# blepping/ComfyUI-sonar

Measured on AMD Instinct MI355X. Metric: noise-latents/sec (SDXL 4x128x128), higher is better.
Workload: dtype f32

## Files before the change

### comfyui-sonar_amd/csrc/power_fft.hip

```cpp
#include "power_core.h"

namespace sonar {

template <int H, int W>
constexpr int plane_min_waves() {
    return (H * W >= 32768 || (H == 256 && W == 64) || (H == 64 && W == 256) || (H == 64 && W == 32)) ? 2 : SONAR_FFT_WAVES;
}

template <int H, int W, int SRC, bool STATS, bool NORM>
__global__ void __launch_bounds__((plane_threads<H, W>()), (plane_min_waves<H, W>())) power_irfft2_kernel(const float* __restrict__ z,
                                                                       const float* __restrict__ filter, float* out,
                                                                       int64_t planes, uint64_t seed, uint64_t stream_id,
                                                                       int64_t plane_offset, int group, int split, double* partials,
                                                                       NormArgs na, StatsAhead sa) {
    kernarg_touch_for(z, filter, out, planes, seed, stream_id, plane_offset, group, split, partials, na, sa);
    using C = PlaneCfg<H, W>;
    constexpr int NT = plane_threads<H, W>();
    constexpr int M = C::M, S = C::S;
    constexpr int RN1 = C::RN1, RN2 = C::RN2;
    constexpr bool FAST = (W == 128) && (H == 128 || H == 64) && (NT == 512) && !SONAR_FFT_TW_LDS;
    constexpr int CN1 = FAST ? H / 8 : C::CN1, CN2 = FAST ? 8 : C::CN2;
    __shared__ c32 A[C::kLdsComplex];
    c32* const T0 = A + H * S;
    c32* const TM = T0 + H;
    c32* const TW = TM + H;
    __shared__ double red[2 * NT / 64];
    __shared__ NormDecision shd;
    __shared__ int edge_seq;
    constexpr bool kSumsInLds = SRC == 2 && STATS && FAST && H == 128;
    __shared__ double sums_lds[kSumsInLds ? 2 * NT : 1];
    const int tid = threadIdx.x;
    if constexpr (kSumsInLds) {
        sums_lds[tid] = 0.0;
        sums_lds[NT + tid] = 0.0;
    }
    int64_t bid = blockIdx.x, nblk = gridDim.x;
    if constexpr (SRC == 1 && NORM && !STATS) {
        static_assert(kStatsBatch * 2 * H <= C::kLdsComplex, "the statistics' edge columns borrow the plane's LDS");
        if (sa.partials) {
            if ((int)blockIdx.x >= sa.main_blocks) {
                power_stats_body<H, W>(filter, planes, seed, sa.stream_id, plane_offset, group, split, sa.partials, bid - sa.main_blocks,
                                       nblk - sa.main_blocks, reinterpret_cast<c32(*)[2][H]>(A), red);
                return;
            }
            nblk = sa.main_blocks;
        }
    }
    constexpr bool GEN = SRC == 1;
    float scale = SRC == 2 ? 1.0f / ((float)H * (float)W) : 1.0f / sqrtf((float)H * (float)W);
    float nm = scale, nc = 0.0f;
    constexpr int NPRE = (NORM && kNPart % NT == 0) ? kNPart / NT : 0;
    [[maybe_unused]] double pre_s[NPRE > 0 ? NPRE : 1], pre_q[NPRE > 0 ? NPRE : 1];
    [[maybe_unused]] bool norm_pending = NORM;
    if constexpr (NORM) {
        if constexpr (NPRE > 0) {
#pragma unroll
            for (int i = 0; i < NPRE; ++i) {
                pre_s[i] = na.partials[2 * (tid + i * NT)];
                pre_q[i] = na.partials[2 * (tid + i * NT) + 1];
            }
        } else {
            const NormDecision dec = decide_norm<NT>(na.partials, kNPart, na.n_total, na.thr_sd, red, &shd);
            const float g = (dec.do_div ? 1.0f / dec.stdv : 1.0f) * na.factor;
            nm = scale * g;
            nc = dec.do_sub ? dec.mean * g : 0.0f;
            norm_pending = false;
        }
    }
    double s = 0.0, q = 0.0;
    for (int j = tid; j < 256; j += NT) TW[j] = c_tw256[j];
#if SONAR_FFT_TW_LDS
    auto tw = [&](int idx, int n, bool) -> c32 { return TW[(idx * (256 / n)) & 255]; };
#else
    auto tw = [&] __device__(int idx, int n, bool uni) -> c32 {
        if (uni) return c_tw256[(__builtin_amdgcn_readfirstlane(idx) * (256 / n)) & 255];
        return TW[(idx * (256 / n)) & 255];
    };
#endif
    const int wv = __builtin_amdgcn_readfirstlane(tid >> 6);
    const int lane = tid & 63;
    c32 ctw[CN1], gtw[RN1], ptw[RN1];
    auto load_twiddles = [&] __device__(int w) {
#pragma unroll
        for (int k1 = 0; k1 < CN1; ++k1) ctw[k1] = c_tw256[((w * k1) * (256 / H)) & 255];
#pragma unroll
        for (int n1 = 0; n1 < RN1; ++n1) gtw[n1] = c_tw256[((RN2 * n1 + w) * (256 / W)) & 255];
#pragma unroll
        for (int k1 = 0; k1 < RN1; ++k1) ptw[k1] = c_tw256[((w * k1) * (256 / M)) & 255];
    };
    if constexpr (FAST) load_twiddles(wv);

#ifdef SONAR_PW_DESYNC
    if (blockIdx.x >= gridDim.x / 2)
        for (int i = 0; i < SONAR_PW_DESYNC; ++i) __builtin_amdgcn_s_sleep(32);
#endif
    [[maybe_unused]] int pidx = 0;
    [[maybe_unused]] int edge_want = 0;
    if (tid == 0) edge_seq = 0;
    for (int64_t unit = bid; unit < (split ? planes : planes / group); unit += nblk) {
    const GroupWalk gw(unit, group, split);
    SpectrumRng rng;
    if constexpr (GEN) {
        rng = spectrum_rng<H, true>(seed, stream_id, plane_offset / group + gw.grp, tid);
        for (int i = 0; i < gw.first; ++i) skip_plane<H, W, true>(rng, tid);
    }
    for (int gp = gw.first; gp < gw.first + gw.count; ++gp) {
        const int64_t plane = gw.grp * group + gp;
        __syncthreads();
        SONAR_STAMP(0);
        int ptid = tid;
        if constexpr (!FAST && H * W >= 4096) asm volatile("" : "+v"(ptid));
        if constexpr (SRC < 2) {
        auto sink = [&](int ky, int kx, c32 v) { (kx == 0 ? T0[ky] : kx == M ? TM[ky] : A[ky * S + kx]) = v; };
        __builtin_amdgcn_s_setprio(0);
        if constexpr (GEN) {
            if constexpr (!(SONAR_PW_SKIP & 1)) fill_plane_gen<H, W, S>(filter, rng, tid, A, T0, TM, (FAST && H == 2 * 64) ? &edge_seq : nullptr);
            if constexpr (FAST && H == 2 * 64 && !(SONAR_PW_SKIP & 1)) {
                edge_want += 2;
                if (tid >= NT - H) {
                    while (__hip_atomic_load(&edge_seq, __ATOMIC_RELAXED, __HIP_MEMORY_SCOPE_WORKGROUP) < edge_want) __builtin_amdgcn_s_sleep(1);
                    __builtin_amdgcn_fence(__ATOMIC_ACQUIRE, "workgroup");
                    const int ky = tid - (NT - H), kn = (H - ky) & (H - 1);
                    const c32 a = T0[ky], an = T0[kn], b = TM[ky], bn = TM[kn];
                    A[ky * S] = make_float2(0.5f * (a.x + an.x) - 0.5f * (b.y - bn.y), 0.5f * (a.y - an.y) + 0.5f * (b.x + bn.x));
                }
            }
        } else fill_plane<H, W>(z, filter, plane, tid, sink);
        __builtin_amdgcn_s_setprio(3);
        SONAR_STAMP(1);
        __syncthreads();
        SONAR_STAMP(2);
        } else {
        constexpr int Wh = M + 1;
        const float* const xin = z + plane * (int64_t)H * W;
#pragma unroll 2
        for (int item = ptid; item < RN1 * H; item += NT) {
            const int k1 = item % RN1, r = item / RN1;
            const int y = (r / CN2) + CN1 * (r % CN2);
            const float* xrow = xin + (int64_t)y * W;
            c32 u[RN2];
#pragma unroll
            for (int k2 = 0; k2 < RN2; ++k2) u[k2] = *reinterpret_cast<const float2*>(xrow + 2 * (k1 + RN1 * k2));
            fdft<RN2>(u);
#pragma unroll
            for (int n2 = 1; n2 < RN2; ++n2) u[n2] = cmulc(u[n2], tw(n2 * k1, M, false));
#pragma unroll
            for (int n2 = 0; n2 < RN2; ++n2) A[r * S + C::rpos(k1, n2)] = u[n2];
        }
        __syncthreads();
        {
            constexpr int ITEMS = (RN2 * H + NT - 1) / NT;
            c32 v[ITEMS][RN1];
#pragma unroll
// ... 191 lines not shown
#pragma unroll
                for (int n1 = 0; n1 < CN1; ++n1) v[n1] = A[(CN2 * n1 + n2) * S + c];
            } else {
#pragma unroll
                for (int n1 = 0; n1 < CN1; ++n1) {
                    const int ky = CN2 * n1 + n2, kn = (H - ky) & (H - 1);
                    const c32 a = T0[ky], an = T0[kn], b = TM[ky], bn = TM[kn];
                    v[n1] = make_float2(0.5f * (a.x + an.x) - 0.5f * (b.y - bn.y), 0.5f * (a.y - an.y) + 0.5f * (b.x + bn.x));
                }
            }
            idft<CN1>(v);
#pragma unroll
            for (int k1 = 1; k1 < CN1; ++k1) v[k1] = cmul(v[k1], tw(n2 * k1, H, M % 64 == 0));
#pragma unroll
            for (int k1 = 0; k1 < CN1; ++k1) A[(CN2 * k1 + n2) * S + c] = v[k1];
        }
        __syncthreads();
SONAR_UNROLL_ITEMS
        for (int item = ptid; item < CN1 * M; item += NT) {
            const int c = item % M, k1 = item / M;
            c32 u[CN2];
#pragma unroll
            for (int n2 = 0; n2 < CN2; ++n2) u[n2] = A[(CN2 * k1 + n2) * S + c];
            idft<CN2>(u);
#pragma unroll
            for (int k2 = 0; k2 < CN2; ++k2) A[(CN2 * k1 + k2) * S + c] = u[k2];
        }
        __syncthreads();
        {
            constexpr int ITEMS = (RN2 * H + NT - 1) / NT;
            c32 g[ITEMS][RN1];
#pragma unroll
            for (int it = 0; it < ITEMS; ++it) {
                const int item = ptid + it * NT;
                if (item < RN2 * H) {
                    const int r = item % H;
                    const int n2 = item / H;
                    const c32* row = A + r * S;
#pragma unroll
                    for (int n1 = 0; n1 < RN1; ++n1) {
                        const int k = RN2 * n1 + n2;
                        c32 xa, xb;
                        if (k == 0) {
                            const c32 p = row[0];
                            xa = make_float2(p.x, 0.0f);
                            xb = make_float2(p.y, 0.0f);
                        } else {
                            xa = row[k];
                            xb = row[M - k];
                        }
                        const c32 e = make_float2(xa.x + xb.x, xa.y - xb.y);
                        const c32 d = make_float2(xa.x - xb.x, xa.y + xb.y);
                        const c32 o = cmul(d, tw(k, W, H % 64 == 0));
                        g[it][n1] = make_float2(e.x - o.y, e.y + o.x);
                    }
                    idft<RN1>(g[it]);
#pragma unroll
                    for (int k1 = 1; k1 < RN1; ++k1) g[it][k1] = cmul(g[it][k1], tw(n2 * k1, M, H % 64 == 0));
                }
                __builtin_amdgcn_sched_barrier(0);
            }
            __syncthreads();
#pragma unroll
            for (int it = 0; it < ITEMS; ++it) {
                const int item = ptid + it * NT;
                if (item < RN2 * H) {
                    const int r = item % H;
                    const int n2 = item / H;
#pragma unroll
                    for (int k1 = 0; k1 < RN1; ++k1) A[r * S + C::rpos(k1, n2)] = g[it][k1];
                }
            }
        }
        __syncthreads();
        }
        if constexpr (NPRE > 0) {
            if (norm_pending) {
                double ps0 = 0.0, pq0 = 0.0;
#pragma unroll
                for (int i = 0; i < NPRE; ++i) {
                    ps0 += pre_s[i];
                    pq0 += pre_q[i];
                }
                const NormDecision dec = decide_from_sums<NT>(ps0, pq0, na.n_total, na.thr_sd, red, &shd);
                const float g = (dec.do_div ? 1.0f / dec.stdv : 1.0f) * na.factor;
                nm = scale * g;
                nc = dec.do_sub ? dec.mean * g : 0.0f;
                norm_pending = false;
            }
        }
        float* const oplane = out + plane * (int64_t)H * W;
        if constexpr (FAST && H == 128) {
            if constexpr (kSumsInLds) {
                double ps_ = 0.0, pq_ = 0.0;
                pipe_row_b<H, W, 8, STATS, NORM>(A, oplane, wv, lane, scale, nm, nc, ps_, pq_);
                sums_lds[tid] += ps_;
                sums_lds[NT + tid] += pq_;
            } else {
                pipe_row_b<H, W, 8, STATS, NORM>(A, oplane, wv, lane, scale, nm, nc, s, q);
            }
            SONAR_STAMP(11);
            ++pidx;
            continue;
        }
        float ps = 0.0f, pq = 0.0f;
SONAR_UNROLL_ITEMS
        for (int item = ptid; item < RN1 * H; item += NT) {
            const int k1 = item % RN1, r = item / RN1;
            const int y = (r / CN2) + CN1 * (r % CN2);
            c32 u[RN2];
#pragma unroll
            for (int n2 = 0; n2 < RN2; ++n2) u[n2] = (SONAR_PW_SKIP & 8) ? make_float2((float)(item + n2), 1.0f) : A[r * S + C::rpos(k1, n2)];
            if constexpr (!(SONAR_PW_SKIP & 8)) idft<RN2>(u);
            float* orow = oplane + (int64_t)y * W;
#pragma unroll
            for (int k2 = 0; k2 < RN2; ++k2) {
                float a, b;
                if constexpr (NORM) {
                    a = __builtin_fmaf(u[k2].x, nm, -nc);
                    b = __builtin_fmaf(u[k2].y, nm, -nc);
                } else {
                    a = u[k2].x * scale;
                    b = u[k2].y * scale;
                }
                if constexpr (!(SONAR_PW_SKIP & 16)) *reinterpret_cast<float2*>(orow + 2 * (k1 + RN1 * k2)) = make_float2(a, b);
                else if (a == 123.456f && b == 654.321f) *reinterpret_cast<float2*>(orow) = make_float2(a, b);
                if constexpr (STATS) {
                    ps += a + b;
                    pq = __builtin_fmaf(a, a, __builtin_fmaf(b, b, pq));
                }
            }
        }
        if constexpr (STATS) {
            s += (double)ps;
            q += (double)pq;
        }
        SONAR_STAMP(11);
        ++pidx;
    }
    }
    if constexpr (kSumsInLds) {
        s = sums_lds[tid];
        q = sums_lds[NT + tid];
    }
    if constexpr (STATS) write_partial<NT>(s, q, partials, red);
}

#ifndef SONAR_PIPE_NT
#define SONAR_PIPE_NT 0
#endif
#ifndef SONAR_PIPE_CHUNKS
#define SONAR_PIPE_CHUNKS 0, 4
#endif
#ifndef SONAR_AHEAD_SPLIT_A
#define SONAR_AHEAD_SPLIT_A 1
#define SONAR_AHEAD_SPLIT_B 3
#endif
#ifndef SONAR_AHEAD_SPLIT_C
#define SONAR_AHEAD_SPLIT_C 2
#define SONAR_AHEAD_SPLIT_D 3
#endif
#ifndef SONAR_AHEAD_PRIO
#define SONAR_AHEAD_PRIO 0
#endif
#ifndef SONAR_PIPE_DECOUPLE
#define SONAR_PIPE_DECOUPLE 0
#endif
__device__ __forceinline__ void team_wait(const int* ctr, int target) {
    while (__builtin_amdgcn_readfirstlane(__hip_atomic_load(ctr, __ATOMIC_RELAXED, __HIP_MEMORY_SCOPE_WORKGROUP)) < target) __builtin_amdgcn_s_sleep(1);
    asm volatile("" ::: "memory");
}
__device__ __forceinline__ void team_barrier(int* ctr, int target, int lane) {
    asm volatile("s_waitcnt lgkmcnt(0)" ::: "memory");
    if (lane == 0) __hip_atomic_fetch_add(ctr, 1, __ATOMIC_RELAXED, __HIP_MEMORY_SCOPE_WORKGROUP);
    team_wait(ctr, target);
}
#ifndef SONAR_PIPE_PRIO_DRAW
#define SONAR_PIPE_PRIO_DRAW 0
#endif
#ifndef SONAR_PIPE_PRIO_FFT
#define SONAR_PIPE_PRIO_FFT 3
#endif
#ifndef SONAR_PIPE_SKIP
#define SONAR_PIPE_SKIP 0
#endif
#ifdef SONAR_PW_TRACE
__device__ unsigned long long g_pipe_trace[256 * 16 * 10 * 4];
#define SONAR_PIPE_STAMP(slot) do { if (lane == 0 && j < 10 && blockIdx.x < 256) g_pipe_trace[((blockIdx.x * 16 + wv_all) * 10 + j) * 4 + (slot)] = __builtin_readcyclecounter(); } while (0)
#else
#define SONAR_PIPE_STAMP(slot) do { } while (0)
#endif

template <int H, int W, int IT0, int IT1>
__device__ __forceinline__ void draw_chunk_regs(SpectrumRng& g, c32 (&v)[H / 8], const float (&wa)[H / 16], const float (&wb)[H / 16]) {
    constexpr int NT = plane_threads<H, W>(), M = W / 2, PAIRS = (H / 2) * M;
    static_assert(PAIRS % NT == 0 && IT0 <= IT1 && IT1 <= PAIRS / NT && NT == 8 * M && PAIRS / NT == H / 16, "slot = (wave n2, column)");
#pragma unroll
    for (int it = IT0; it < IT1; ++it) {
        const uint32_t ra = g.R.next();
        const uint32_t rb = g.R.next();
        const uint32_t t = g.T.next();
        if constexpr (SONAR_PIPE_SKIP & 2) {
            v[it] = make_float2(wa[it] + (float)ra, wb[it]);
            v[it + H / 16] = make_float2(wb[it] + (float)t, wa[it] + (float)rb);
        } else {
            v[it] = drawn_weighted(ra, angle_lo(t), wa[it]);
            v[it + H / 16] = drawn_weighted(rb, angle_hi(t), wb[it]);
        }
    }
}
template <int H, int W, int IT0, int IT1>
__device__ __forceinline__ void draw_chunk_signs(const float* __restrict__ filter, int tid, c32 (&v)[H / 8]) {
    constexpr int NT = plane_threads<H, W>(), M = W / 2, Wh = M + 1, LM = draw_shift<W>();
#pragma unroll
    for (int it = IT0; it < IT1; ++it) {
        const int p = tid + it * NT, pos = (p >> LM) * Wh + 1 + (p & (M - 1));
        if (filter[pos] < 0.0f) v[it] = make_float2(-v[it].x, -v[it].y);
        if (filter[pos + (H / 2) * Wh] < 0.0f) v[it + H / 16] = make_float2(-v[it + H / 16].x, -v[it + H / 16].y);
    }
}

template <int H, int W, int NW>
__device__ __forceinline__ void pipe_col_b(const c32* X, c32* Y, int w, int lane) {
    constexpr int S = PlaneCfg<H, W>::S, CN1 = H / 8, CN2 = 8, ITEMS = CN1 / NW;
    static_assert(CN1 % NW == 0, "whole items per wave");
    c32 u[ITEMS][CN2];
#pragma unroll
    for (int it = 0; it < ITEMS; ++it) {
#pragma unroll
        for (int n2 = 0; n2 < CN2; ++n2) u[it][n2] = X[(CN2 * (w + NW * it) + n2) * S + lane];
    }
    __builtin_amdgcn_sched_barrier(0);
#pragma unroll
    for (int it = 0; it < ITEMS; ++it) {
        idft<CN2>(u[it]);
#pragma unroll
        for (int k2 = 0; k2 < CN2; ++k2) Y[(CN2 * (w + NW * it) + k2) * S + lane] = u[it][k2];
    }
}

template <int W>
__device__ __forceinline__ RowATw<W> row_a_twiddles(int w) {
    static_assert(W == 128, "c_rowa_tw128");
    int cls = w < 6 ? (w >> 1) : w - 3;
    asm volatile("" : "+s"(cls));
    const c32* t = c_rowa_tw128[cls];
    RowATw<W> r;
#pragma unroll
    for (int i = 0; i < 8; ++i) {
        r.g[i] = t[i];
        r.p[i] = t[8 + i];
    }
    return r;
}
__device__ __forceinline__ c32 cconj(c32 a) { return make_float2(a.x, -a.y); }
__device__ __forceinline__ c32 cmul_conj(c32 a, c32 b) {
    const v2f A = vv(a), B = vv(b);
    return cc(__builtin_elementwise_fma(A.yx, v2f{B.y, -B.y}, A * B.xx));
}

template <int H, int W, int NW, int LAYOUT>
__device__ __forceinline__ void pipe_row_a(const c32* Y, c32* X, int w, int lane) {
    using C = PlaneCfg<H, W>;
    constexpr bool INPLACE = LAYOUT == kRowsInPlace, SWZ = LAYOUT == kRowsSwizzled;
    auto swz_base = [](int res) {
        int b = (res & 1) + 16 * (res >> 1);
        if constexpr (SWZ) asm volatile("" : "+s"(b));
        return b;
    };
    auto cin = [&](int n1, int res, int base) { return SWZ ? 2 * n1 + base : 8 * n1 + res; };
    auto cout = [&](int k1, int res, int base) { return SWZ ? 2 * k1 + base : 8 * res + k1; };
    static_assert(!SWZ || (C::kRowSwizzle && C::rpos(3, 5) == 2 * 3 + 1 + 16 * 2), "cin / cout restate PlaneCfg::rpos");
    const RowATw<W> tw = row_a_twiddles<W>(__builtin_amdgcn_readfirstlane(w));
    constexpr int M = C::M, S = C::S, RN1 = C::RN1, RN2 = C::RN2;
    static_assert(H == 128 && RN1 == 8 && RN2 == 8 && NW == 8, "three residue pairs x two row halves + two self-mirrored residues x all rows");
    auto pair = [&](c32 xa, c32 xb, c32 g, c32& plus, c32& minus_conj) {
        const c32 xc = cconj(xb);
        const c32 s = cadd(xa, xc), d = cmul(csub(xa, xc), g);
        plus = cadd_i(s, d);
        minus_conj = cc(vv(d).yx + v2f{s.x, -s.y});
    };
    if (w < 6) {
        const int a = 1 + (w >> 1), b = 8 - a, r = lane + 64 * (w & 1);
        const int ba = swz_base(a), bb = swz_base(b);
        const c32* row = Y + r * S;
        c32 xa[8], xb[8];
#pragma unroll
        for (int n1 = 0; n1 < 8; ++n1) {
            xa[n1] = row[cin(n1, a, ba)];
            xb[n1] = row[cin(7 - n1, b, bb)];
        }
        __builtin_amdgcn_sched_barrier(0);
        c32 ga[8], tb[8];
#pragma unroll
        for (int n1 = 0; n1 < 8; ++n1) {
            c32 m;
            pair(xa[n1], xb[n1], tw.g[n1], ga[n1], m);
            tb[(8 - n1) & 7] = m;
        }
        idft<8>(ga);
        idft<8>(tb);
#pragma unroll
        for (int k1 = 1; k1 < 8; ++k1) ga[k1] = cmul(ga[k1], tw.p[k1]);
#pragma unroll
        for (int k1 = 1; k1 < 8; ++k1) tb[k1] = cmul_conj(tb[k1], tw.p[k1]);
        if constexpr (INPLACE) __syncthreads();
        c32* orow = X + r * S;
#pragma unroll
        for (int k1 = 0; k1 < 8; ++k1) orow[cout(k1, a, ba)] = ga[k1];
#pragma unroll
        for (int k1 = 0; k1 < 8; ++k1) orow[cout(k1, b, bb)] = tb[k1];
    } else {
        const bool zero = w == 6;
        const int a = zero ? 0 : 4, ba = swz_base(a);
        c32 x[2][8];
#pragma unroll
        for (int it = 0; it < 2; ++it) {
            const c32* row = Y + (lane + 64 * it) * S;
#pragma unroll
            for (int n1 = 0; n1 < 8; ++n1) x[it][n1] = row[cin(n1, a, ba)];
        }
        __builtin_amdgcn_sched_barrier(0);
        c32 g[2][8];
#pragma unroll
        for (int it = 0; it < 2; ++it) {
            if (zero) {
                const c32 p = x[it][0];
                {
                    const c32 xa = make_float2(p.x, 0.0f), xc = make_float2(p.y, -0.0f);
                    g[it][0] = cadd_i(cadd(xa, xc), cmul(csub(xa, xc), tw.g[0]));
                }
                {
                    const c32 xa = x[it][4], xc = cconj(xa);
                    g[it][4] = cadd_i(cadd(xa, xc), cmul(csub(xa, xc), tw.g[4]));
                }
#pragma unroll
                for (int n1 = 1; n1 < 4; ++n1) {
                    c32 m;
                    pair(x[it][n1], x[it][8 - n1], tw.g[n1], g[it][n1], m);
                    g[it][8 - n1] = m;
                }
            } else {
#pragma unroll
// ... 205 lines not shown
        xch->q[16 * wo + lane] = make_float2(__builtin_fmaf(a.x, p.x, a.y * pn.x), __builtin_fmaf(a.x, p.y, -(a.y * pn.y)));
    }
    __builtin_amdgcn_fence(__ATOMIC_RELEASE, "wavefront");
    __builtin_amdgcn_wave_barrier();
    __builtin_amdgcn_fence(__ATOMIC_ACQUIRE, "wavefront");
    if (lane == 0) {
        const float4* const src = reinterpret_cast<const float4*>(xch->q + 16 * wo);
#pragma unroll
        for (int n1 = 0; n1 < N; n1 += 2) {
            const float4 t = src[n1 / 2];
            v[n1] = make_float2(t.x, t.y);
            v[n1 + 1] = make_float2(t.z, t.w);
        }
    }
    SONAR_STAMP(9);
    idft<N>(v);
    const c32* const t = c_cola_tw128[wo];
#pragma unroll
    for (int k1 = 1; k1 < N; ++k1) v[k1] = cmul(v[k1], t[k1]);
    SONAR_STAMP(10);
#pragma unroll
    for (int k1 = 0; k1 < N; ++k1) A[(8 * k1 + w) * S + lane] = v[k1];
}

#ifndef SONAR_SF_FILTER_EARLY
#define SONAR_SF_FILTER_EARLY 1
#endif
#ifndef SONAR_SF_PREFETCH
#define SONAR_SF_PREFETCH 1
#endif
#ifndef SONAR_SF_WIDE
#define SONAR_SF_WIDE 1
#endif
template <int H, int W, bool STATS>
__global__ void __launch_bounds__(512, 4) spectral_filter128_kernel(const float* __restrict__ x, const float* __restrict__ filter, float* out, int64_t planes,
                                                                     double* partials) {
    kernarg_touch_for(x, filter, out, planes, partials);
    using C = PlaneCfg<H, W>;
    constexpr int NT = 512, M = C::M, S = C::S, Wh = C::Wh, RN1 = C::RN1, RN2 = C::RN2, CN1 = H / 8, CN2 = 8;
    static_assert(H == 128 && W == 128 && RN1 == 8 && RN2 == 8 && plane_threads<H, W>() == NT, "8 waves, 8 x 8 rows, 16 x 8 columns");
    __shared__ __attribute__((aligned(16))) c32 A[H * S];
    __shared__ __attribute__((aligned(16))) SfExchange<H> xch;
    __shared__ c32 TW[M];
    __shared__ double red[2 * NT / 64];
    const int tid = threadIdx.x, wv = __builtin_amdgcn_readfirstlane(tid >> 6);
    for (int j = tid; j < M; j += NT) TW[j] = c_tw256[j * (256 / M)];
    for (int i = tid; i < H; i += NT) {
        const int ky = 8 * (i & 15) + (i >> 4), kn = (H - ky) & (H - 1);
        const float g0 = 0.5f * (filter[ky * Wh] + filter[kn * Wh]), gm = 0.5f * (filter[ky * Wh + M] + filter[kn * Wh + M]);
        xch.wgt[i] = make_float2(0.5f * (g0 + gm), 0.5f * (g0 - gm));
    }
    const float scale = 0.5f / ((float)H * (float)W);
    __shared__ double sums[STATS ? 2 * NT : 1];
    if constexpr (STATS) {
        sums[tid] = 0.0;
        sums[NT + tid] = 0.0;
    }
    [[maybe_unused]] int pidx = 0;
    c32 u[2][RN2];
    constexpr bool WIDE = SONAR_SF_WIDE != 0;
    auto request = [&](int64_t plane, int t) {
        if constexpr (WIDE) {
            const int r = t >> 2, y = (r / CN2) + CN1 * (r % CN2);
            const float* xrow = x + plane * (int64_t)H * W + (int64_t)y * W + 4 * (t & 3);
#pragma unroll
            for (int k2 = 0; k2 < RN2; ++k2) {
                const float4 v = *reinterpret_cast<const float4*>(xrow + 2 * RN1 * k2);
                u[0][k2] = make_float2(v.x, v.y);
                u[1][k2] = make_float2(v.z, v.w);
            }
        } else {
            const int k1 = t & 7;
#pragma unroll
            for (int it = 0; it < 2; ++it) {
                const int r = (t >> 3) + 64 * it, y = (r / CN2) + CN1 * (r % CN2);
                const float* xrow = x + plane * (int64_t)H * W + (int64_t)y * W;
#pragma unroll
                for (int k2 = 0; k2 < RN2; ++k2) u[it][k2] = *reinterpret_cast<const float2*>(xrow + 2 * (k1 + RN1 * k2));
            }
        }
    };
    auto finish = [&](int64_t plane, int lane) {
        pipe_col_b<H, W, 8>(A, A, wv, lane);
        __syncthreads();
        SONAR_STAMP(5);
        pipe_row_a<H, W, 8, kRowsSwizzled>(A, A, wv, lane);
        __syncthreads();
        SONAR_STAMP(6);
        double ps = 0.0, pq = 0.0;
        pipe_row_b<H, W, 8, STATS, false, kRowsSwizzled>(A, out + plane * (int64_t)H * W, wv, lane, scale, scale, 0.0f, ps, pq);
        if constexpr (STATS) {
            sums[tid] += ps;
            sums[NT + tid] += pq;
        }
        SONAR_STAMP(11);
        ++pidx;
    };
    int64_t plane = blockIdx.x;
    if (plane >= planes) return;
    if (SONAR_SF_PREFETCH) request(plane, tid);
    for (;;) {
        __syncthreads();
        SONAR_STAMP(0);
        int ptid = tid;
        asm volatile("" : "+v"(ptid));
        const int lane = ptid & 63;
        if (!SONAR_SF_PREFETCH) request(plane, ptid);
        {
#pragma unroll
            for (int it = 0; it < 2; ++it) {
                const int k1 = WIDE ? 2 * (ptid & 3) + it : ptid & 7, r = WIDE ? ptid >> 2 : (ptid >> 3) + 64 * it;
                fdft<RN2>(u[it]);
#pragma unroll
                for (int n2 = 1; n2 < RN2; ++n2) u[it][n2] = cmulc(u[it][n2], TW[(n2 * k1) & (M - 1)]);
#pragma unroll
                for (int n2 = 0; n2 < RN2; ++n2) A[r * S + C::rpos(k1, n2)] = u[it][n2];
            }
        }
        __syncthreads();
        SONAR_STAMP(1);
        sf_row_a_split<H, W>(A, wv, lane);
        __syncthreads();
        SONAR_STAMP(2);
        float f[CN1];
        if (SONAR_SF_FILTER_EARLY) sf_filter_values<H, W>(filter, wv, lane, f);
        sf_col_b<H, W>(A, wv, lane);
        __syncthreads();
        SONAR_STAMP(3);
        if (!SONAR_SF_FILTER_EARLY) sf_filter_values<H, W>(filter, wv, lane, f);
        sf_col_a_filter_col_a<H, W>(A, &xch, f, wv, lane, pidx);
        __syncthreads();
        SONAR_STAMP(4);
        const int64_t next = plane + gridDim.x;
        if (next >= planes) {
            finish(plane, lane);
            break;
        }
        if (SONAR_SF_PREFETCH) request(next, ptid);
        finish(plane, lane);
        plane = next;
    }
    if constexpr (STATS) write_partial<NT>(sums[tid], sums[NT + tid], partials, red);
}

template <int H, int W>
struct TeamStats {
    static constexpr int NT = plane_threads<H, W>(), M = W / 2, Wh = M + 1, LM = draw_shift<W>(), PAIRS = (H / 2) * M, ITER = draw_iters<H, W>();
    float wgt[2 * ITER], prod[2 * ITER];
    float f0, fm;
    SpectrumRng rng;
    double s, q;
    int planes_in_unit;

    __device__ __forceinline__ void begin(const float* __restrict__ filter, uint64_t seed, uint64_t stream_id, int64_t plane_offset, int group,
                                          const GroupWalk& gw, int tid, c32* edge, const float* wa = nullptr, const float* wb = nullptr) {
#pragma unroll
        for (int it = 0; it < ITER; ++it) {
            const int p = tid + it * NT, ky = p >> LM, kx = 1 + (p & (M - 1));
            const bool live = p < PAIRS && kx < M;
            if (wa) {
                wgt[it] = live ? wa[it] : 0.0f;
                wgt[it + ITER] = live ? wb[it] : 0.0f;
            } else {
                wgt[it] = filter_weight(live ? filter[ky * Wh + kx] : 0.0f);
                wgt[it + ITER] = filter_weight(live ? filter[(ky + H / 2) * Wh + kx] : 0.0f);
            }
            prod[it] = 1.0f;
            prod[it + ITER] = 1.0f;
        }
        f0 = tid < H ? filter[tid * Wh] : 0.0f;
        fm = tid < H ? filter[tid * Wh + M] : 0.0f;
        s = 0.0;
        q = 0.0;
        planes_in_unit = gw.count;
        rng = spectrum_rng<H, false>(seed, stream_id, plane_offset / group + gw.grp, tid);
        for (int i = 0; i < gw.first; ++i) skip_plane<H, W, false>(rng, tid);
        if (tid < H) {
            for (int b = 0; b < gw.count; ++b) {
                const uint32_t r0 = rng.E.next();
                const uint32_t rm = rng.E.next();
                const uint32_t t = rng.E.next();
                edge[(2 * b) * H + tid] = drawn_elem(r0, angle_lo(t), f0);
                edge[(2 * b + 1) * H + tid] = drawn_elem(rm, angle_hi(t), fm);
            }
        }
    }
    __device__ __forceinline__ void radii(int b0, int b1, int tid) {
        for (int b = b0; b < min(b1, planes_in_unit); ++b) {
#pragma unroll
            for (int it = 0; it < ITER; ++it) {
                const uint32_t ra = rng.R.next();
                const uint32_t rb = rng.R.next();
                prod[it] *= 2.0f - unit_mantissa(ra);
                prod[it + ITER] *= 2.0f - unit_mantissa(rb);
            }
        }
#pragma unroll
        for (int it = 0; it < 2 * ITER; ++it) asm volatile("" : "+v"(prod[it]));
    }
    __device__ __forceinline__ void products() {
        float acc = 0.0f;
#pragma unroll
        for (int it = 0; it < 2 * ITER; ++it) acc = __builtin_fmaf(wgt[it], __builtin_amdgcn_logf(prod[it]), acc);
        q += 2.0 * (double)acc;
    }
    __device__ __forceinline__ void edges_and_wave_sums(const c32* edge, int tid, double* sred) {
        for (int b = 0; b < planes_in_unit; ++b) {
            float e = 0.0f;
            if (tid < H) {
                const int ky = tid, kn = (H - ky) & (H - 1);
                const c32 a = edge[(2 * b) * H + ky], an = edge[(2 * b) * H + kn], c = edge[(2 * b + 1) * H + ky], cn = edge[(2 * b + 1) * H + kn];
                const float ar = 0.5f * (a.x + an.x), ai = 0.5f * (a.y - an.y), br = 0.5f * (c.x + cn.x), bi = 0.5f * (c.y - cn.y);
                e += (ar * ar + ai * ai) + (br * br + bi * bi);
                if (ky == 0) s += (double)(sqrtf((float)H * (float)W) * ar);
            }
            q += (double)e;
        }
        const double ws = wave_sum(s), wq = wave_sum(q);
        if ((tid & 63) == 0) {
            sred[tid >> 6] = ws;
            sred[NT / 64 + (tid >> 6)] = wq;
        }
    }
    static __device__ __forceinline__ void store(const double* sred, int tid, double* partials_next, int64_t slot) {
        if (tid == 0) {
            double ss = 0.0, qq = 0.0;
#pragma unroll
            for (int i = 0; i < NT / 64; ++i) {
                ss += sred[i];
                qq += sred[NT / 64 + i];
            }
            partials_next[2 * slot] = ss;
            partials_next[2 * slot + 1] = qq;
        }
    }
};

template <int IT0, int IT1, int N>
__device__ __forceinline__ void pin_chunk(c32 (&v)[N]) {
#pragma unroll
    for (int it = IT0; it < IT1; ++it) {
        asm volatile("" : "+v"(v[it].x), "+v"(v[it].y), "+v"(v[it + N / 2].x), "+v"(v[it + N / 2].y));
    }
}

#ifndef SONAR_PIPE_KERNARG_TOUCH
#define SONAR_PIPE_KERNARG_TOUCH 1
#endif
template <int H, int W, bool STATS, bool NORM>
__global__ void __launch_bounds__(1024) power_pipe_kernel(const float* __restrict__ filter, float* out, int64_t planes, uint64_t seed,
                                                          uint64_t stream_id, int64_t plane_offset, int group, int split, double* partials,
                                                          NormArgs na, uint64_t next_stream, double* partials_next) {
#if SONAR_PIPE_KERNARG_TOUCH
    kernarg_touch_for(filter, out, planes, seed, stream_id, plane_offset, group, split, partials, na, next_stream, partials_next);
#endif
    using C = PlaneCfg<H, W>;
    constexpr int NT = 512, NALL = 1024;
    static_assert(plane_threads<H, W>() == NT && W == 128 && H == 128, "one 8-wave team per plane, slot = one radix-16 column item");
    constexpr int M = C::M, S = C::S, Wh = M + 1, RN1 = C::RN1, RN2 = C::RN2, CN1 = H / 8, CN2 = 8, ITER = draw_iters<H, W>();
    constexpr int LM = draw_shift<W>();
    constexpr int kChunk[2] = {SONAR_PIPE_CHUNKS};
    constexpr int E0 = kChunk[0], E1 = E0 + kChunk[1];
    static_assert(E1 <= ITER && ITER == CN1 / 2, "chunks of whole pair iterations");
    constexpr int BUF = H * S;
    __shared__ c32 PLANES[2 * BUF];
    __shared__ c32 EDGE[3 * H];
    __shared__ uint4 SEED_RT[NT];
    static_assert(sizeof(uint4) * NT >= sizeof(c32) * 2 * H * kAheadMaxGroup, "edge columns of a look-ahead unit fit the seed area");
    __shared__ double sred[2 * NT / 64];
    __shared__ double red[2 * NALL / 64];
    __shared__ int tbar, dbar;
    if constexpr (SONAR_PIPE_DECOUPLE) {
        if (threadIdx.x == 0) {
            tbar = 0;
            dbar = 0;
        }
        __syncthreads();
    }
    __shared__ NormDecision shd;
    const int wv_all = __builtin_amdgcn_readfirstlane((int)threadIdx.x >> 6);
    const bool drawer = wv_all >= NT / 64;
    const int tid = threadIdx.x & (NT - 1), lane = threadIdx.x & 63, wv = wv_all & (NT / 64 - 1);
    const int64_t nunits = split ? planes : planes / group;
    const int64_t group0 = plane_offset / group;
    const int per_unit = split ? 1 : group;
    const int64_t my_units = (int64_t)blockIdx.x < nunits ? (nunits - blockIdx.x + gridDim.x - 1) / gridDim.x : 0;
    const int n = (int)(my_units * per_unit);
    const bool ahead = partials_next != nullptr && nunits <= 2 * (int64_t)gridDim.x;
    const float scale = 1.0f / sqrtf((float)H * (float)W);
    float nm = scale, nc = 0.0f;
    static_assert(!NORM || kNPart == NALL, "one partial pair per thread");
    [[maybe_unused]] double pre_s = 0.0, pre_q = 0.0;
    if constexpr (NORM) {
        pre_s = na.partials[2 * threadIdx.x];
        pre_q = na.partials[2 * threadIdx.x + 1];
    }
    auto leave_wave_sums = [&]() {
        if constexpr (NORM) {
            const double ws = wave_sum(pre_s), wq = wave_sum(pre_q);
            if (lane == 0) {
                red[wv_all] = ws;
                red[NALL / 64 + wv_all] = wq;
            }
        }
    };
    auto decide_in_wave0 = [&]() {
        if constexpr (NORM) {
            if (wv_all == 0) {
                double ss = 0.0, qq = 0.0;
#pragma unroll
                for (int i = 0; i < NALL / 64; ++i) {
                    ss += red[i];
                    qq += red[NALL / 64 + i];
                }
                const NormDecision dec = decision_from_totals(ss, qq, na.n_total, na.thr_sd);
                if (lane == 0) shd = dec;
            }
        }
    };
    auto pick_up_decision = [&]() {
        if constexpr (NORM) {
            const NormDecision dec = shd;
            const float g = (dec.do_div ? 1.0f / dec.stdv : 1.0f) * na.factor;
            nm = scale * g;
            nc = dec.do_sub ? dec.mean * g : 0.0f;
        }
    };
    double s = 0.0, q = 0.0;
    if (drawer) {
        __builtin_amdgcn_s_setprio(SONAR_PIPE_PRIO_DRAW);
        const c32* const Q = EDGE + 2 * H;
        SpectrumRng rng;
        float wa[ITER], wb[ITER];
        bool neg = false;
#pragma unroll
        for (int it = 0; it < ITER; ++it) {
            const int p = tid + it * NT, pos = (p >> LM) * Wh + 1 + (p & (M - 1));
            const float fa = filter[pos], fb = filter[pos + (H / 2) * Wh];
            wa[it] = filter_weight(fa);
            wb[it] = filter_weight(fb);
            neg = neg || fa < 0.0f || fb < 0.0f;
        }
        const bool wave_neg = __builtin_amdgcn_ballot_w64(neg) != 0;
        c32 ctw[CN1];
#pragma unroll
        for (int k1 = 0; k1 < CN1; ++k1) ctw[k1] = c_tw256[((wv * k1) * (256 / H)) & 255];
        const int col = (lane + 1) & (M - 1);
        int64_t unit = blockIdx.x;
        int gp = 0;
        for (int j = 0; j < n; ++j) {
            c32* const A = PLANES + (j & 1) * BUF;
            c32 v[CN1];
            SONAR_PIPE_STAMP(0);
            if (gp == 0) {
                const GroupWalk gw(unit, group, split);
                if (j == per_unit) {
                    const uint4 rt = SEED_RT[tid];
                    rng.R = Mwc{rt.x, rt.y};
                    rng.T = Mwc{rt.z, rt.w};
                } else {
                    rng = spectrum_seed<true>(seed, stream_id, group0 + gw.grp, tid, false);
                }
                for (int i = 0; i < gw.first; ++i) skip_plane<H, W, true, false>(rng, tid);
            }
            if constexpr (SONAR_PIPE_DECOUPLE) {
                draw_chunk_regs<H, W, 0, ITER>(rng, v, wa, wb);
                if (wave_neg) draw_chunk_signs<H, W, 0, ITER>(filter, tid, v);
                pin_chunk<0, ITER>(v);
                SONAR_PIPE_STAMP(1);
                SONAR_PIPE_STAMP(2);
                team_wait(&tbar, 2 * (NT / 64) * (j + 1));
            } else {
            draw_chunk_regs<H, W, 0, E0>(rng, v, wa, wb);
            if (wave_neg) draw_chunk_signs<H, W, 0, E0>(filter, tid, v);
            pin_chunk<0, E0>(v);
            SONAR_PIPE_STAMP(1);
            __syncthreads();
            draw_chunk_regs<H, W, E0, E1>(rng, v, wa, wb);
            if (wave_neg) draw_chunk_signs<H, W, E0, E1>(filter, tid, v);
            pin_chunk<E0, E1>(v);
            SONAR_PIPE_STAMP(2);
            __syncthreads();
            draw_chunk_regs<H, W, E1, ITER>(rng, v, wa, wb);
            if (wave_neg) draw_chunk_signs<H, W, E1, ITER>(filter, tid, v);
            }
            if (lane == M - 1) {
#pragma unroll
                for (int n1 = 0; n1 < CN1; ++n1) v[n1] = Q[CN2 * n1 + wv];
            }
            idft<CN1>(v);
#pragma unroll
            for (int k1 = 1; k1 < CN1; ++k1) v[k1] = cmul(v[k1], ctw[k1]);
#pragma unroll
            for (int k1 = 0; k1 < CN1; ++k1) A[(CN2 * k1 + wv) * S + col] = v[k1];
            if (++gp == per_unit) {
                gp = 0;
                unit += gridDim.x;
            }
            if (j == 0) leave_wave_sums();
            SONAR_PIPE_STAMP(3);
            __syncthreads();
        }
        [[maybe_unused]] const int j = n;
        SONAR_PIPE_STAMP(0);
        if (ahead && my_units == 2) {
            TeamStats<H, W> ts;
            c32* const edge = reinterpret_cast<c32*>(SEED_RT);
            const GroupWalk gw((int64_t)blockIdx.x + gridDim.x, group, split);
            ts.begin(filter, seed, next_stream, plane_offset, group, gw, tid, edge, wa, wb);
            ts.radii(0, SONAR_AHEAD_SPLIT_A, tid);
            SONAR_PIPE_STAMP(1);
            if constexpr (SONAR_PIPE_DECOUPLE) team_barrier(&dbar, NT / 64, lane);
            else __syncthreads();
            ts.radii(SONAR_AHEAD_SPLIT_A, SONAR_AHEAD_SPLIT_B, tid);
            SONAR_PIPE_STAMP(2);
            if constexpr (!SONAR_PIPE_DECOUPLE) __syncthreads();
            ts.radii(SONAR_AHEAD_SPLIT_B, 4, tid);
            ts.products();
            ts.edges_and_wave_sums(edge, tid, sred);
            SONAR_PIPE_STAMP(3);
            __syncthreads();
        } else {
            SONAR_PIPE_STAMP(1);
            if constexpr (!SONAR_PIPE_DECOUPLE) __syncthreads();
            SONAR_PIPE_STAMP(2);
            if constexpr (!SONAR_PIPE_DECOUPLE) __syncthreads();
            SONAR_PIPE_STAMP(3);
            __syncthreads();
        }
    } else {
        __builtin_amdgcn_s_setprio(SONAR_PIPE_PRIO_FFT);
        int64_t unit = blockIdx.x;
        int gp = 0;
        c32* const T0 = EDGE;
        c32* const TM = EDGE + H;
        c32* const Q = EDGE + 2 * H;
        const float f0 = tid < H ? filter[tid * Wh] : 0.0f, fm = tid < H ? filter[tid * Wh + M] : 0.0f;
        Mwc rngE{0, 1}, rngE2{0, 1};
        int64_t eunit = blockIdx.x;
        int egp = 0;
        auto draw_edges = [&](int je) {
            if (tid < H && je < n) {
                if (egp == 0) {
                    const GroupWalk gw(eunit, group, split);
                    rngE = je == per_unit ? rngE2 : spectrum_seed<false>(seed, stream_id, group0 + gw.grp, tid, true).E;
                    for (int i = 0; i < 3 * gw.first; ++i) rngE.next();
                }
                const uint32_t r0 = rngE.next();
                const uint32_t rm = rngE.next();
                const uint32_t t = rngE.next();
                T0[tid] = drawn_elem(r0, angle_lo(t), f0);
                TM[tid] = drawn_elem(rm, angle_hi(t), fm);
                if (++egp == per_unit) {
                    egp = 0;
                    eunit += gridDim.x;
                }
            }
        };
        auto pack_edges = [&](int je) {
            if (tid >= NT - H && je < n) {
                const int ky = tid - (NT - H), kn = (H - ky) & (H - 1);
                const c32 a = T0[ky], an = T0[kn], b = TM[ky], bn = TM[kn];
                Q[ky] = make_float2(0.5f * (a.x + an.x) - 0.5f * (b.y - bn.y), 0.5f * (a.y - an.y) + 0.5f * (b.x + bn.x));
            }
        };
        if (n > per_unit) {
            const GroupWalk gw(unit + gridDim.x, group, split);
            const SpectrumRng g2 = spectrum_rng<H, true>(seed, stream_id, group0 + gw.grp, tid);
            SEED_RT[tid] = make_uint4(g2.R.x, g2.R.c, g2.T.x, g2.T.c);
            rngE2 = g2.E;
        }
        [[maybe_unused]] const int j = 0;
        SONAR_PIPE_STAMP(0);
        int tb = 0;
        auto exchange = [&]() {
            if constexpr (SONAR_PIPE_DECOUPLE) team_barrier(&tbar, (NT / 64) * ++tb, lane);
            else __syncthreads();
        };
        if (ahead && my_units >= 1) {
            TeamStats<H, W> ts;
            c32* const edge = PLANES + BUF;
            const GroupWalk gw(unit, group, split);
            if (blockIdx.x == 0)
                for (int64_t slot = nunits + tid; slot < kNPart; slot += NT) {
                    partials_next[2 * slot] = 0.0;
                    partials_next[2 * slot + 1] = 0.0;
                }
            __builtin_amdgcn_s_setprio(SONAR_AHEAD_PRIO);
            draw_edges(0);
            ts.begin(filter, seed, next_stream, plane_offset, group, gw, tid, edge);
            ts.radii(0, SONAR_AHEAD_SPLIT_C, tid);
            SONAR_PIPE_STAMP(1);
            exchange();
            pack_edges(0);
            ts.radii(SONAR_AHEAD_SPLIT_C, SONAR_AHEAD_SPLIT_D, tid);
            SONAR_PIPE_STAMP(2);
            exchange();
            ts.radii(SONAR_AHEAD_SPLIT_D, 4, tid);
            ts.products();
            ts.edges_and_wave_sums(edge, tid, sred);
            leave_wave_sums();
            SONAR_PIPE_STAMP(3);
            __syncthreads();
            TeamStats<H, W>::store(sred, tid, partials_next, unit);
            __builtin_amdgcn_s_setprio(SONAR_PIPE_PRIO_FFT);
        } else {
            draw_edges(0);
            SONAR_PIPE_STAMP(1);
            exchange();
            pack_edges(0);
            SONAR_PIPE_STAMP(2);
            exchange();
            leave_wave_sums();
            SONAR_PIPE_STAMP(3);
            __syncthreads();
        }
        for (int j = 1; j <= n; ++j) {
            constexpr int NW = 8;
            const bool work = j >= 1;
            c32* const X = PLANES + ((j + 1) & 1) * BUF;
            c32* const Y = PLANES + (j & 1) * BUF;
            SONAR_PIPE_STAMP(0);
            if (work && !(SONAR_PIPE_SKIP & 16)) pipe_col_b<H, W, NW>(X, Y, wv, lane);
            draw_edges(j);
            if (j == 1) decide_in_wave0();
            SONAR_PIPE_STAMP(1);
            exchange();
            if (work && !(SONAR_PIPE_SKIP & 8)) pipe_row_a<H, W, NW>(Y, X, wv, lane);
            pack_edges(j);
            SONAR_PIPE_STAMP(2);
            exchange();
            if (work) {
                if (j == 1) pick_up_decision();
                const GroupWalk gw(unit, group, split);
                float* const oplane = out + (gw.grp * group + gw.first + gp) * (int64_t)H * W;
                pipe_row_b<H, W, NW, STATS, NORM>(X, oplane, wv, lane, scale, nm, nc, s, q);
                if (++gp == per_unit) {
                    gp = 0;
                    unit += gridDim.x;
                }
            }
            SONAR_PIPE_STAMP(3);
            __syncthreads();
        }
    }
    if (ahead) {
        __syncthreads();
        if (drawer && my_units == 2) TeamStats<H, W>::store(sred, tid, partials_next, (int64_t)blockIdx.x + gridDim.x);
    }
    if constexpr (STATS) write_partial<NALL>(s, q, partials, red);
}

template <int H, int W>
__device__ __forceinline__ void power_stats_body(const float* __restrict__ filter, int64_t planes, uint64_t seed, uint64_t stream_id,
                                                 int64_t plane_offset, int group, int split, double* partials, int64_t bid, int64_t nb,
                                                 c32 (*EDGE)[2][H] , double* red) {
    constexpr int NT = plane_threads<H, W>(), M = W / 2, Wh = M + 1;
    constexpr int NB = kStatsBatch;
    const int tid = threadIdx.x;
    double s = 0.0, q = 0.0;
    auto edge_terms = [&](int p) {
        float edge = 0.0f;
        for (int ky = tid; ky < H; ky += NT) {
            const int kn = (H - ky) & (H - 1);
            const c32 a = EDGE[p][0][ky], an = EDGE[p][0][kn], b = EDGE[p][1][ky], bn = EDGE[p][1][kn];
            const float ar = 0.5f * (a.x + an.x), ai = 0.5f * (a.y - an.y), br = 0.5f * (b.x + bn.x), bi = 0.5f * (b.y - bn.y);
            edge += (ar * ar + ai * ai) + (br * br + bi * bi);
            if (ky == 0) s += (double)(sqrtf((float)H * (float)W) * ar);
        }
        q += (double)edge;
    };
    constexpr int LM = draw_shift<W>(), PAIRS = (H / 2) * M, ITER = draw_iters<H, W>();
    float wgt[2 * ITER];
#pragma unroll
    for (int it = 0; it < ITER; ++it) {
        const int p = tid + it * NT, ky = p >> LM, kx = 1 + (p & (M - 1));
        const bool live = p < PAIRS && kx < M;
        wgt[it] = filter_weight(live ? filter[ky * Wh + kx] : 0.0f);
        wgt[it + ITER] = filter_weight(live ? filter[(ky + H / 2) * Wh + kx] : 0.0f);
    }
    const float f0 = tid < H ? filter[tid * Wh] : 0.0f, fm = tid < H ? filter[tid * Wh + M] : 0.0f;
    for (int64_t unit = bid; unit < (split ? planes : planes / group); unit += nb) {
        const GroupWalk gw(unit, group, split);
        SpectrumRng rng = spectrum_rng<H, false>(seed, stream_id, plane_offset / group + gw.grp, tid);
        for (int i = 0; i < gw.first; ++i) skip_plane<H, W, false>(rng, tid);
        for (int g0 = 0; g0 < gw.count; g0 += NB) {
            const int cnt = min(NB, gw.count - g0);
            float prod[2 * ITER];
#pragma unroll
            for (int it = 0; it < 2 * ITER; ++it) prod[it] = 1.0f;
            for (int b = 0; b < cnt; ++b) {
                draw_plane<H, W, false>(
                    rng, tid,
                    [&](uint32_t r0, uint32_t rm, uint32_t t) {
                        EDGE[b][0][tid] = drawn_elem(r0, angle_lo(t), f0);
                        EDGE[b][1][tid] = drawn_elem(rm, angle_hi(t), fm);
                    },
                    [&](int it, int, uint32_t ra, uint32_t rb, uint32_t) {
                        prod[it] *= 2.0f - unit_mantissa(ra);
                        prod[it + ITER] *= 2.0f - unit_mantissa(rb);
                    });
            }
            float acc = 0.0f;
#pragma unroll
            for (int it = 0; it < 2 * ITER; ++it) acc = __builtin_fmaf(wgt[it], __builtin_amdgcn_logf(prod[it]), acc);
            q += 2.0 * (double)acc;
            __syncthreads();
            for (int b = 0; b < cnt; ++b) edge_terms(b);
            __syncthreads();
        }
    }
    write_partial_at<NT>(s, q, partials, red, (int)bid, (int)nb);
}

template <int H, int W>
__global__ void __launch_bounds__((plane_threads<H, W>())) power_stats_kernel(const float* __restrict__ filter, int64_t planes, uint64_t seed,
                                                                   uint64_t stream_id, int64_t plane_offset, int group, int split,
                                                                   double* partials) {
    kernarg_touch_for(filter, planes, seed, stream_id, plane_offset, group, split, partials);
    __shared__ c32 EDGE[kStatsBatch][2][H];
    __shared__ double red[2 * plane_threads<H, W>() / 64];
    power_stats_body<H, W>(filter, planes, seed, stream_id, plane_offset, group, split, partials, blockIdx.x, gridDim.x, EDGE, red);
}

template <int H, int W>
__global__ void __launch_bounds__((plane_threads<H, W>())) power_spectrum_kernel(float* zout, int64_t planes, uint64_t seed, uint64_t stream_id,
                                                                      int64_t plane_offset, int group, int split) {
    kernarg_touch_for(zout, planes, seed, stream_id, plane_offset, group, split);
    constexpr int M = W / 2, Wh = M + 1, NC = H * Wh;
    const int tid = threadIdx.x;
    for (int64_t unit = blockIdx.x; unit < (split ? planes : planes / group); unit += gridDim.x) {
        const GroupWalk gw(unit, group, split);
        SpectrumRng rng = spectrum_rng<H, true>(seed, stream_id, plane_offset / group + gw.grp, tid);
// ... 334 lines not shown
```

Before: 12.71 million.

## Issue filter and partials loads early to overlap with RNG seeding in pipe kernel

Splits filter-weight loading from the transform so global loads of the filter and normalization partials are issued before the RNG seeding and skip work, with sched barriers and register pins to keep that order. The first drawer iteration is peeled with its own chunk split (default 3,3), and the ahead-stats radii split points are shifted. The goal is to hide global load latency at kernel start behind independent integer RNG work. In exchange, more registers stay live across the seeding phase, which may add register pressure.

```diff
diff --git a/comfyui-sonar_amd/csrc/power_fft.hip b/comfyui-sonar_amd/csrc/power_fft.hip
--- a/comfyui-sonar_amd/csrc/power_fft.hip
+++ b/comfyui-sonar_amd/csrc/power_fft.hip
@@ -1,4 +1,6 @@
 #include "power_core.h"
+
+#include <type_traits>
 
 namespace sonar {
 
@@ -496,13 +498,16 @@
 #ifndef SONAR_PIPE_CHUNKS
 #define SONAR_PIPE_CHUNKS 0, 4
 #endif
+#ifndef SONAR_PIPE_CHUNKS0
+#define SONAR_PIPE_CHUNKS0 3, 3
+#endif
 #ifndef SONAR_AHEAD_SPLIT_A
 #define SONAR_AHEAD_SPLIT_A 1
 #define SONAR_AHEAD_SPLIT_B 3
 #endif
 #ifndef SONAR_AHEAD_SPLIT_C
-#define SONAR_AHEAD_SPLIT_C 2
-#define SONAR_AHEAD_SPLIT_D 3
+#define SONAR_AHEAD_SPLIT_C 3
+#define SONAR_AHEAD_SPLIT_D 4
 #endif
 #ifndef SONAR_AHEAD_PRIO
 #define SONAR_AHEAD_PRIO 0
@@ -531,8 +536,10 @@
 #ifdef SONAR_PW_TRACE
 __device__ unsigned long long g_pipe_trace[256 * 16 * 10 * 4];
 #define SONAR_PIPE_STAMP(slot) do { if (lane == 0 && j < 10 && blockIdx.x < 256) g_pipe_trace[((blockIdx.x * 16 + wv_all) * 10 + j) * 4 + (slot)] = __builtin_readcyclecounter(); } while (0)
+#define SONAR_PIPE_STAMP_ENTRY() do { if ((threadIdx.x & 63) == 0 && blockIdx.x < 256) g_pipe_trace[((blockIdx.x * 16 + (threadIdx.x >> 6)) * 10 + 9) * 4] = __builtin_readcyclecounter(); } while (0)
 #else
 #define SONAR_PIPE_STAMP(slot) do { } while (0)
+#define SONAR_PIPE_STAMP_ENTRY() do { } while (0)
 #endif
 
 template <int H, int W, int IT0, int IT1>
@@ -1044,22 +1051,17 @@
     double s, q;
     int planes_in_unit;
 
-    __device__ __forceinline__ void begin(const float* __restrict__ filter, uint64_t seed, uint64_t stream_id, int64_t plane_offset, int group,
-                                          const GroupWalk& gw, int tid, c32* edge, const float* wa = nullptr, const float* wb = nullptr) {
+    __device__ __forceinline__ void request(const float* __restrict__ filter, int tid) {
 #pragma unroll
         for (int it = 0; it < ITER; ++it) {
             const int p = tid + it * NT, ky = p >> LM, kx = 1 + (p & (M - 1));
             const bool live = p < PAIRS && kx < M;
-            if (wa) {
-                wgt[it] = live ? wa[it] : 0.0f;
-                wgt[it + ITER] = live ? wb[it] : 0.0f;
-            } else {
-                wgt[it] = filter_weight(live ? filter[ky * Wh + kx] : 0.0f);
-                wgt[it + ITER] = filter_weight(live ? filter[(ky + H / 2) * Wh + kx] : 0.0f);
-            }
-            prod[it] = 1.0f;
-            prod[it + ITER] = 1.0f;
-        }
+            wgt[it] = live ? filter[ky * Wh + kx] : 0.0f;
+            wgt[it + ITER] = live ? filter[(ky + H / 2) * Wh + kx] : 0.0f;
+        }
+    }
+    __device__ __forceinline__ void begin(const float* __restrict__ filter, uint64_t seed, uint64_t stream_id, int64_t plane_offset, int group,
+                                          const GroupWalk& gw, int tid, c32* edge, const float* wa = nullptr, const float* wb = nullptr) {
         f0 = tid < H ? filter[tid * Wh] : 0.0f;
         fm = tid < H ? filter[tid * Wh + M] : 0.0f;
         s = 0.0;
@@ -1067,6 +1069,22 @@
         planes_in_unit = gw.count;
         rng = spectrum_rng<H, false>(seed, stream_id, plane_offset / group + gw.grp, tid);
         for (int i = 0; i < gw.first; ++i) skip_plane<H, W, false>(rng, tid);
+        asm volatile("" : "+v"(rng.R.x), "+v"(rng.R.c), "+v"(rng.E.x), "+v"(rng.E.c));
+        __builtin_amdgcn_sched_barrier(0);
+#pragma unroll
+        for (int it = 0; it < ITER; ++it) {
+            const int p = tid + it * NT, kx = 1 + (p & (M - 1));
+            const bool live = p < PAIRS && kx < M;
+            if (wa) {
+                wgt[it] = live ? wa[it] : 0.0f;
+                wgt[it + ITER] = live ? wb[it] : 0.0f;
+            } else {
+                wgt[it] = filter_weight(wgt[it]);
+                wgt[it + ITER] = filter_weight(wgt[it + ITER]);
+            }
+            prod[it] = 1.0f;
+            prod[it + ITER] = 1.0f;
+        }
         if (tid < H) {
             for (int b = 0; b < gw.count; ++b) {
                 const uint32_t r0 = rng.E.next();
@@ -1146,14 +1164,14 @@
 #if SONAR_PIPE_KERNARG_TOUCH
     kernarg_touch_for(filter, out, planes, seed, stream_id, plane_offset, group, split, partials, na, next_stream, partials_next);
 #endif
+    SONAR_PIPE_STAMP_ENTRY();
     using C = PlaneCfg<H, W>;
     constexpr int NT = 512, NALL = 1024;
     static_assert(plane_threads<H, W>() == NT && W == 128 && H == 128, "one 8-wave team per plane, slot = one radix-16 column item");
     constexpr int M = C::M, S = C::S, Wh = M + 1, RN1 = C::RN1, RN2 = C::RN2, CN1 = H / 8, CN2 = 8, ITER = draw_iters<H, W>();
     constexpr int LM = draw_shift<W>();
-    constexpr int kChunk[2] = {SONAR_PIPE_CHUNKS};
-    constexpr int E0 = kChunk[0], E1 = E0 + kChunk[1];
-    static_assert(E1 <= ITER && ITER == CN1 / 2, "chunks of whole pair iterations");
+    constexpr int kChunk[2] = {SONAR_PIPE_CHUNKS}, kChunk0[2] = {SONAR_PIPE_CHUNKS0};
+    static_assert(ITER == CN1 / 2, "a slot's pair iterations are the inputs of its radix-16 item");
     constexpr int BUF = H * S;
     __shared__ c32 PLANES[2 * BUF];
     __shared__ c32 EDGE[3 * H];
@@ -1183,10 +1201,12 @@
     float nm = scale, nc = 0.0f;
     static_assert(!NORM || kNPart == NALL, "one partial pair per thread");
     [[maybe_unused]] double pre_s = 0.0, pre_q = 0.0;
-    if constexpr (NORM) {
-        pre_s = na.partials[2 * threadIdx.x];
-        pre_q = na.partials[2 * threadIdx.x + 1];
-    }
+    auto request_partials = [&]() {
+        if constexpr (NORM) {
+            pre_s = na.partials[2 * threadIdx.x];
+            pre_q = na.partials[2 * threadIdx.x + 1];
+        }
+    };
     auto leave_wave_sums = [&]() {
         if constexpr (NORM) {
             const double ws = wave_sum(pre_s), wq = wave_sum(pre_q);
@@ -1222,29 +1242,45 @@
     if (drawer) {
         __builtin_amdgcn_s_setprio(SONAR_PIPE_PRIO_DRAW);
         const c32* const Q = EDGE + 2 * H;
-        SpectrumRng rng;
         float wa[ITER], wb[ITER];
-        bool neg = false;
 #pragma unroll
         for (int it = 0; it < ITER; ++it) {
             const int p = tid + it * NT, pos = (p >> LM) * Wh + 1 + (p & (M - 1));
-            const float fa = filter[pos], fb = filter[pos + (H / 2) * Wh];
-            wa[it] = filter_weight(fa);
-            wb[it] = filter_weight(fb);
-            neg = neg || fa < 0.0f || fb < 0.0f;
-        }
-        const bool wave_neg = __builtin_amdgcn_ballot_w64(neg) != 0;
+            wa[it] = filter[pos];
+            wb[it] = filter[pos + (H / 2) * Wh];
+        }
+        request_partials();
+        __builtin_amdgcn_sched_barrier(0);
         c32 ctw[CN1];
 #pragma unroll
         for (int k1 = 0; k1 < CN1; ++k1) ctw[k1] = c_tw256[((wv * k1) * (256 / H)) & 255];
         const int col = (lane + 1) & (M - 1);
         int64_t unit = blockIdx.x;
         int gp = 0;
-        for (int j = 0; j < n; ++j) {
+        SpectrumRng rng;
+        {
+            const GroupWalk gw(unit, group, split);
+            rng = spectrum_seed<true>(seed, stream_id, group0 + gw.grp, tid, false);
+            for (int i = 0; i < gw.first; ++i) skip_plane<H, W, true, false>(rng, tid);
+        }
+        asm volatile("" : "+v"(rng.R.x), "+v"(rng.R.c), "+v"(rng.T.x), "+v"(rng.T.c));
+        __builtin_amdgcn_sched_barrier(0);
+        bool neg = false;
+#pragma unroll
+        for (int it = 0; it < ITER; ++it) {
+            const float fa = wa[it], fb = wb[it];
+            wa[it] = filter_weight(fa);
+            wb[it] = filter_weight(fb);
+            neg = neg || fa < 0.0f || fb < 0.0f;
+        }
+        const bool wave_neg = __builtin_amdgcn_ballot_w64(neg) != 0;
+        auto iteration = [&](auto k0, auto k1, const int j) __attribute__((always_inline)) {
+            constexpr int K0 = decltype(k0)::value, K1 = K0 + decltype(k1)::value;
+            static_assert(K1 <= ITER, "chunks of whole pair iterations");
             c32* const A = PLANES + (j & 1) * BUF;
             c32 v[CN1];
             SONAR_PIPE_STAMP(0);
-            if (gp == 0) {
+            if (gp == 0 && j != 0) {
                 const GroupWalk gw(unit, group, split);
                 if (j == per_unit) {
                     const uint4 rt = SEED_RT[tid];
@@ -1263,18 +1299,18 @@
                 SONAR_PIPE_STAMP(2);
                 team_wait(&tbar, 2 * (NT / 64) * (j + 1));
             } else {
-            draw_chunk_regs<H, W, 0, E0>(rng, v, wa, wb);
-            if (wave_neg) draw_chunk_signs<H, W, 0, E0>(filter, tid, v);
-            pin_chunk<0, E0>(v);
+            draw_chunk_regs<H, W, 0, K0>(rng, v, wa, wb);
+            if (wave_neg) draw_chunk_signs<H, W, 0, K0>(filter, tid, v);
+            pin_chunk<0, K0>(v);
             SONAR_PIPE_STAMP(1);
             __syncthreads();
-            draw_chunk_regs<H, W, E0, E1>(rng, v, wa, wb);
-            if (wave_neg) draw_chunk_signs<H, W, E0, E1>(filter, tid, v);
-            pin_chunk<E0, E1>(v);
+            draw_chunk_regs<H, W, K0, K1>(rng, v, wa, wb);
+            if (wave_neg) draw_chunk_signs<H, W, K0, K1>(filter, tid, v);
+            pin_chunk<K0, K1>(v);
             SONAR_PIPE_STAMP(2);
             __syncthreads();
-            draw_chunk_regs<H, W, E1, ITER>(rng, v, wa, wb);
-            if (wave_neg) draw_chunk_signs<H, W, E1, ITER>(filter, tid, v);
+            draw_chunk_regs<H, W, K1, ITER>(rng, v, wa, wb);
+            if (wave_neg) draw_chunk_signs<H, W, K1, ITER>(filter, tid, v);
             }
             if (lane == M - 1) {
 #pragma unroll
@@ -1292,7 +1328,9 @@
             if (j == 0) leave_wave_sums();
             SONAR_PIPE_STAMP(3);
             __syncthreads();
-        }
+        };
+        if (n > 0) iteration(std::integral_constant<int, kChunk0[0]>(), std::integral_constant<int, kChunk0[1]>(), 0);
+        for (int j = 1; j < n; ++j) iteration(std::integral_constant<int, kChunk[0]>(), std::integral_constant<int, kChunk[1]>(), j);
         [[maybe_unused]] const int j = n;
         SONAR_PIPE_STAMP(0);
         if (ahead && my_units == 2) {
@@ -1328,6 +1366,7 @@
         c32* const TM = EDGE + H;
         c32* const Q = EDGE + 2 * H;
         const float f0 = tid < H ? filter[tid * Wh] : 0.0f, fm = tid < H ? filter[tid * Wh + M] : 0.0f;
+        request_partials();
         Mwc rngE{0, 1}, rngE2{0, 1};
         int64_t eunit = blockIdx.x;
         int egp = 0;
@@ -1356,6 +1395,9 @@
                 Q[ky] = make_float2(0.5f * (a.x + an.x) - 0.5f * (b.y - bn.y), 0.5f * (a.y - an.y) + 0.5f * (b.x + bn.x));
             }
         };
+        const bool stats0 = ahead && my_units >= 1;
+        TeamStats<H, W> ts;
+        if (stats0) ts.request(filter, tid);
         if (n > per_unit) {
             const GroupWalk gw(unit + gridDim.x, group, split);
             const SpectrumRng g2 = spectrum_rng<H, true>(seed, stream_id, group0 + gw.grp, tid);
@@ -1369,8 +1411,7 @@
             if constexpr (SONAR_PIPE_DECOUPLE) team_barrier(&tbar, (NT / 64) * ++tb, lane);
             else __syncthreads();
         };
-        if (ahead && my_units >= 1) {
-            TeamStats<H, W> ts;
+        if (stats0) {
             c32* const edge = PLANES + BUF;
             const GroupWalk gw(unit, group, split);
             if (blockIdx.x == 0)
```

After: 12.81 million, median of 3. No clear change (+0.9%).
